# mantasu/face-crop-plus

Hardware: AMD Instinct MI355X
Metric: faces/sec end-to-end (detect+align+crop) (higher is better)
Workload: dtype f16x3; 1 GPU; RetinaFace detect + 5-pt align/crop, batch=32/GPU synthetic 1024x1024 RGB, strategy=largest, det_threshold=0.6, output 256x256, detector on 2 HIP streams x 16 images; global_batch=32, image_size=1024, parallelism=dp1

## Files before the change

### face-crop-plus_amd/csrc/fcp_conv_common.h

```cpp
#pragma once
#include <type_traits>
#include "fcp_common.h"
#include "fcp_hip.h"

typedef float f32x16 __attribute__((ext_vector_type(16)));
typedef float f32x4 __attribute__((ext_vector_type(4)));


constexpr int FCP_AUX_A = 0;
constexpr int FCP_AUX_B = 0;

namespace fcp_conv {

constexpr int BM = 128;
constexpr int BK = 32;

struct ConvK {
  const float* in;
  const float* w;
  const float* bias;
  float* out;
  const float* res1;
  const float* res2;
  int n, in_h, in_w, ph, pw, cin, in_ld, in_up2;
  int cout, kh, kw, stride, pad, out_h, out_w, out_ld;
  int pad_h;
  int M, ktiles, ctiles, wrow;
  float act_slope, alpha, alpha2;
  int res1_pre, res1_ld, res1_h, res1_w, res1_resize, res2_ld;
  float res1_sh, res1_sw;
  int grid_m, grid_n, vec_ok;
  unsigned in_bytes, w_bytes;
  const float* wscale;
  int in_fmt, out_fmt, res1_fmt, res2_fmt;
  const float* in2;
  unsigned in2_bytes;
  int csplit, in2_ld, ph2, pw2, stride2;
  int nt_store;
  int balance, cu_budget;
  int mfull, tail_rows, round_size;
  int big_tiles;
  int big_persist;
};


struct TapPiece {
  unsigned base, mask;
};

template <bool CIN4>
__device__ __forceinline__ TapPiece make_tap_piece(const ConvK& p, unsigned pbase, int hi0, int wi0, unsigned chan_off) {
  TapPiece t;
  t.base = ((pbase + (unsigned)(hi0 * p.pw + wi0)) * (unsigned)p.in_ld + chan_off) * 4u;
  t.mask = 0u;
  const int taps = CIN4 ? p.kh : p.kh * p.kw;
  for (int q = 0; q < taps; ++q) {
    const int kh_i = CIN4 ? q : q / p.kw;
    const int kw_i = CIN4 ? 0 : q - kh_i * p.kw;
    const bool ok = (unsigned)(hi0 + kh_i) < (unsigned)p.in_h && (unsigned)(wi0 + kw_i) < (unsigned)p.in_w;
    t.mask |= ok ? (1u << q) : 0u;
  }
  return t;
}

typedef unsigned int u32x4_t __attribute__((ext_vector_type(4)));
typedef _Float16 f16x2_t __attribute__((ext_vector_type(2)));
typedef _Float16 f16x8 __attribute__((ext_vector_type(8)));


__device__ __forceinline__ int xcd_tile_order(int nb, int bid) {
  const int q8 = nb >> 3, r8 = nb & 7, xcd = bid & 7;
  return (xcd < r8 ? xcd * (q8 + 1) : r8 * (q8 + 1) + (xcd - r8) * q8) + (bid >> 3);
}

template <typename M>
__device__ __forceinline__ void conv_out_pixel(const ConvK& p, M m, int hw, int& ni, int& ho, int& wo) {
  ni = (int)(m / hw);
  const int rem = (int)(m - (M)ni * hw);
  ho = rem / p.out_w;
  wo = rem - ho * p.out_w;
}

struct ConvRow {
  int ni;
  unsigned pbase;
  int hi0, wi0;
  unsigned base2;
};
__device__ __forceinline__ ConvRow conv_row(const ConvK& p, int m, int m_end, int hw, unsigned chan_off2) {
  ConvRow r = {0, 0u, -(1 << 28), 0, 0xFFFFFFFFu};
  if (m < m_end) {
    int ho, wo;
    conv_out_pixel(p, m, hw, r.ni, ho, wo);
    r.pbase = (unsigned)(r.ni * p.ph * p.pw);
    r.hi0 = ho * p.stride - p.pad_h;
    r.wi0 = wo * p.stride - p.pad;
    if (p.in2 != nullptr)
      r.base2 = (((unsigned)(r.ni * p.ph2 + ho * p.stride2) * (unsigned)p.pw2 + (unsigned)(wo * p.stride2)) * (unsigned)p.in2_ld + chan_off2) * 4u;
  }
  return r;
}

struct RowPiece {
  unsigned pbase;
  int hi0, wi0;
  int col;
  unsigned chan_off;
  TapPiece tp;
};
template <bool CIN4>
__device__ __forceinline__ RowPiece make_row_piece(const ConvK& p, const ConvRow& r, int col, unsigned chan_off) {
  RowPiece c = {r.pbase, r.hi0, r.wi0, CIN4 ? col : 0, CIN4 ? 0u : chan_off, {0u, 0u}};
  c.tp = make_tap_piece<CIN4>(p, c.pbase, c.hi0, c.wi0 + c.col, c.chan_off);
  return c;
}

struct TapWalk {
  int tap = 0, kh_i = 0, kw_i = 0, c0 = 0;
  template <bool CIN4>
  __device__ __forceinline__ void advance(const ConvK& p) {
    ++tap;
    if (CIN4) {
      ++kh_i;
    } else if (++kw_i >= p.kw) {
      kw_i = 0;
      if (++kh_i >= p.kh) { kh_i = 0; tap = 0; c0 += BK; }
    }
  }
};

template <bool CIN4, bool UP2, int NP>
__device__ __forceinline__ void set_tap(const ConvK& p, const TapWalk& t, const RowPiece (&pc)[NP], unsigned (&rowoff)[NP]) {
  if (UP2 && p.in_up2) {
#pragma unroll
    for (int i = 0; i < NP; ++i) {
      int hi = pc[i].hi0 + t.kh_i;
      int wi = pc[i].wi0 + (CIN4 ? pc[i].col : t.kw_i);
      const bool ok = (unsigned)hi < (unsigned)p.in_h && (unsigned)wi < (unsigned)p.in_w;
      hi >>= 1; wi >>= 1;
      const unsigned pix = pc[i].pbase + (unsigned)(hi * p.pw + wi);
      rowoff[i] = ok ? (pix * (unsigned)p.in_ld + pc[i].chan_off) * 4u : 0xFFFFFFFFu;
    }
  } else {
    const unsigned tapoff = (unsigned)((t.kh_i * p.pw + t.kw_i) * p.in_ld) * 4u;
#pragma unroll
    for (int i = 0; i < NP; ++i) rowoff[i] = ((pc[i].tp.mask >> t.tap) & 1u) ? pc[i].tp.base + tapoff : 0xFFFFFFFFu;
  }
}
template <bool CIN4, bool UP2, int NP>
__device__ __forceinline__ void next_tap(const ConvK& p, TapWalk& t, const RowPiece (&pc)[NP], unsigned (&rowoff)[NP]) {
  t.advance<CIN4>(p);
  set_tap<CIN4, UP2>(p, t, pc, rowoff);
}

__device__ __forceinline__ f32x4 buf_load16(__amdgpu_buffer_rsrc_t rsrc, unsigned voff) {
  return __builtin_bit_cast(f32x4, __builtin_amdgcn_raw_buffer_load_b128(rsrc, (int)voff, 0, 0));
}
__device__ __forceinline__ u32x4_t buf_load16u(__amdgpu_buffer_rsrc_t rsrc, unsigned voff) {
  return __builtin_bit_cast(u32x4_t, __builtin_amdgcn_raw_buffer_load_b128(rsrc, (int)voff, 0, 0));
}

template <int STEP, int A_LD, int B_LD>
__device__ __forceinline__ void dma_slice(const ConvK& p, __amdgpu_buffer_rsrc_t rs_in, __amdgpu_buffer_rsrc_t rs_in2, __amdgpu_buffer_rsrc_t rs_w,
                                          char* a, char* b, const unsigned (&rowoff)[A_LD], const unsigned (&base2)[A_LD],
                                          const unsigned (&woff)[B_LD], int c0, int kt) {
  constexpr int ROWB = 128;
  if (c0 >= p.csplit) {
#pragma unroll
    for (int i = 0; i < A_LD; ++i) {
      const unsigned ro = base2[i];
      __builtin_amdgcn_raw_ptr_buffer_load_lds(rs_in2, (__attribute__((address_space(3))) void*)(a + STEP * i * ROWB), 16,
                                               (int)(ro == 0xFFFFFFFFu ? 0xFFFFFFFFu : ro + (unsigned)((c0 - p.csplit) * 4)), 0, 0, FCP_AUX_A);
    }
  } else {
#pragma unroll
    for (int i = 0; i < A_LD; ++i) {
      const unsigned ro = rowoff[i];
      __builtin_amdgcn_raw_ptr_buffer_load_lds(rs_in, (__attribute__((address_space(3))) void*)(a + STEP * i * ROWB), 16,
                                               (int)(ro == 0xFFFFFFFFu ? 0xFFFFFFFFu : ro + (unsigned)(c0 * 4)), 0, 0, FCP_AUX_A);
    }
  }
#pragma unroll
  for (int i = 0; i < B_LD; ++i)
    __builtin_amdgcn_raw_ptr_buffer_load_lds(rs_w, (__attribute__((address_space(3))) void*)(b + STEP * i * ROWB), 16,
                                             (int)(woff[i] + (unsigned)(kt * BK * 4)), 0, 0, FCP_AUX_B);
}

__device__ __forceinline__ int swz(int row) { return ((row >> 1) & 7) ^ ((row & 1) << 2); }

__device__ __forceinline__ void frag_offsets(int lane, int (&offH)[2], int (&offL)[2]) {
  const int rsw = (((lane & 31) >> 1) & 7) ^ ((lane & 1) << 2);
  const int half = lane >> 5;
#pragma unroll
  for (int s = 0; s < 2; ++s) {
    offH[s] = ((2 * s + half) ^ rsw) << 4;
    offL[s] = ((4 + 2 * s + half) ^ rsw) << 4;
  }
}

template <int IMM>
__device__ __forceinline__ f16x8 lds_read128i(unsigned addr) {
  f16x8 v;
  asm volatile("ds_read_b128 %0, %1 offset:%2" : "=v"(v) : "v"(addr), "n"(IMM));
  return v;
}

template <int TM, int TN>
__device__ __forceinline__ void clear_acc(f32x16 (&acc)[TM][TN]) {
#pragma unroll
  for (int i = 0; i < TM; ++i)
#pragma unroll
    for (int j = 0; j < TN; ++j)
#pragma unroll
      for (int e = 0; e < 16; ++e) acc[i][j][e] = 0.f;
}

template <int HI>
__device__ __forceinline__ float fcp_mix_sum(unsigned h, unsigned l) {
  float r;
  const float one = 1.0f;
  if constexpr (HI) asm("v_fma_mix_f32 %0, %1, %2, %3 op_sel:[1,0,1] op_sel_hi:[1,0,1]" : "=v"(r) : "v"(h), "s"(one), "v"(l));
  else asm("v_fma_mix_f32 %0, %1, %2, %3 op_sel:[0,0,0] op_sel_hi:[1,0,1]" : "=v"(r) : "v"(h), "s"(one), "v"(l));
  return r;
}
template <int HI>
__device__ __forceinline__ float fcp_mix_diff(float x, unsigned h) {
  float r;
  const float minus_one = -1.0f;
  if constexpr (HI) asm("v_fma_mix_f32 %0, %1, %2, %3 op_sel:[1,0,0] op_sel_hi:[1,0,0]" : "=v"(r) : "v"(h), "s"(minus_one), "v"(x));
  else asm("v_fma_mix_f32 %0, %1, %2, %3 op_sel:[0,0,0] op_sel_hi:[1,0,0]" : "=v"(r) : "v"(h), "s"(minus_one), "v"(x));
  return r;
}

__device__ __forceinline__ void split8(const f32x4& x0, const f32x4& x1, u32x4_t& hi, u32x4_t& lo) {
  const float x[8] = {x0[0], x0[1], x0[2], x0[3], x1[0], x1[1], x1[2], x1[3]};
#pragma unroll
  for (int q = 0; q < 4; ++q) {
    const unsigned hu = __builtin_bit_cast(unsigned, __builtin_amdgcn_cvt_pkrtz(x[2 * q], x[2 * q + 1]));
    const float r0 = fcp_mix_diff<0>(x[2 * q], hu);
    const float r1 = fcp_mix_diff<1>(x[2 * q + 1], hu);
    hi[q] = hu;
    lo[q] = __builtin_bit_cast(unsigned, __builtin_amdgcn_cvt_pkrtz(r0, r1));
  }
}
__device__ __forceinline__ void split2(float x0, float x1, unsigned& hu, unsigned& lu) {
  hu = __builtin_bit_cast(unsigned, __builtin_amdgcn_cvt_pkrtz(x0, x1));
  lu = __builtin_bit_cast(unsigned, __builtin_amdgcn_cvt_pkrtz(fcp_mix_diff<0>(x0, hu), fcp_mix_diff<1>(x1, hu)));
}
__device__ __forceinline__ void join8(const u32x4_t& hi, const u32x4_t& lo, float (&x)[8]) {
#pragma unroll
  for (int q = 0; q < 4; ++q) {
    const unsigned hu = hi[q], lu = lo[q];
    x[2 * q] = fcp_mix_sum<0>(hu, lu);
    x[2 * q + 1] = fcp_mix_sum<1>(hu, lu);
  }
}
__device__ __forceinline__ long split_chan_off(int c) { return (long)(c >> 5) * 128 + (c & 31) * 2; }

__device__ __forceinline__ void load8(const float* base, long pix, int ld, int c, int fmt, float (&x)[8]) {
  if (fmt == 1) {
    const char* pb = reinterpret_cast<const char*>(base) + pix * ld * 4 + split_chan_off(c);
    join8(*reinterpret_cast<const u32x4_t*>(pb), *reinterpret_cast<const u32x4_t*>(pb + 64), x);
  } else {
    const f32x4 a = *reinterpret_cast<const f32x4*>(base + pix * ld + c);
    const f32x4 b = *reinterpret_cast<const f32x4*>(base + pix * ld + c + 4);
    x[0] = a[0]; x[1] = a[1]; x[2] = a[2]; x[3] = a[3]; x[4] = b[0]; x[5] = b[1]; x[6] = b[2]; x[7] = b[3];
  }
}

__device__ __forceinline__ void pack8(const float (&v)[8], int fmt, u32x4_t& a, u32x4_t& b) {
  if (fmt == 1) {
    split8(f32x4{v[0], v[1], v[2], v[3]}, f32x4{v[4], v[5], v[6], v[7]}, a, b);
  } else {
    a = __builtin_bit_cast(u32x4_t, f32x4{v[0], v[1], v[2], v[3]});
    b = __builtin_bit_cast(u32x4_t, f32x4{v[4], v[5], v[6], v[7]});
  }
}
__device__ __forceinline__ void store8(float* base, long pix, int ld, int c, int fmt, int nt, const u32x4_t& a, const u32x4_t& b) {
  if (fmt == 1) {
    char* ob = reinterpret_cast<char*>(base) + pix * ld * 4 + split_chan_off(c);
    if (nt) {
      __builtin_nontemporal_store(a, reinterpret_cast<u32x4_t*>(ob));
      __builtin_nontemporal_store(b, reinterpret_cast<u32x4_t*>(ob + 64));
    } else {
      *reinterpret_cast<u32x4_t*>(ob) = a;
      *reinterpret_cast<u32x4_t*>(ob + 64) = b;
    }
  } else {
    float* dst = base + pix * ld + c;
    *reinterpret_cast<u32x4_t*>(dst) = a;
    *reinterpret_cast<u32x4_t*>(dst + 4) = b;
  }
}
__device__ __forceinline__ void pack_store8(float* base, long pix, int ld, int c, int fmt, int nt, const float (&v)[8]) {
  u32x4_t a, b;
  if (fmt == 1) {
    pack8(v, 1, a, b);
    store8(base, pix, ld, c, 1, nt, a, b);
  } else {
    pack8(v, 0, a, b);
    store8(base, pix, ld, c, 0, 0, a, b);
  }
}

__device__ __forceinline__ float conv_scale_bias(float acc, float ws, float b) { return acc * ws + b; }

struct ConvEpi {
  bool res1, res1_pre, res2;
  float act_slope, alpha, alpha2;
};
template <typename E>
__device__ __forceinline__ float conv_finish(const E e, float x, float r1, float r2) {
  if (e.res1 && e.res1_pre) x += r1;
  x = x >= 0.f ? x : x * e.act_slope;
  x = x * e.alpha;
  if (e.res1 && !e.res1_pre) x += r1;
  if (e.res2) x = x * e.alpha2 + r2;
  return x;
}
template <typename E>
__device__ __forceinline__ float conv_value(const E& e, float acc, float ws, float b, float r1, float r2) {
  return conv_finish(e, conv_scale_bias(acc, ws, b), r1, r2);
}
__device__ __forceinline__ float conv_finish_relu(float x) { return conv_finish(ConvEpi{false, false, false, 0.f, 1.f, 1.f}, x, 0.f, 0.f); }
__device__ __forceinline__ float conv_finish_relu(float x, float r1) { return conv_finish(ConvEpi{true, true, false, 0.f, 1.f, 1.f}, x, r1, 0.f); }
__device__ __forceinline__ float conv_value_relu(float acc, float ws, float b) { return conv_finish_relu(conv_scale_bias(acc, ws, b)); }

__device__ __forceinline__ long res1_pixel(const ConvK& p, long m, int hw) {
  int ni, ho, wo;
  conv_out_pixel(p, m, hw, ni, ho, wo);
  int sh = (int)floorf(ho * p.res1_sh);
  int sw = (int)floorf(wo * p.res1_sw);
  sh = sh < p.res1_h - 1 ? sh : p.res1_h - 1;
  sw = sw < p.res1_w - 1 ? sw : p.res1_w - 1;
  return ((long)ni * p.res1_h + sh) * p.res1_w + sw;
}

__device__ __forceinline__ constexpr int mfma_c_row(int rr, int half) { return (rr & 3) + 8 * (rr >> 2) + 4 * half; }

template <int BN, int TM, int TN, int WTM, int WTN>
__device__ __forceinline__ void stage_acc_tile(const f32x16 (&acc)[TM][TN], float* Cs, int lane, int wm, int wn) {
  const int half = lane >> 5;
#pragma unroll
  for (int i = 0; i < TM; ++i)
#pragma unroll
    for (int j = 0; j < TN; ++j)
#pragma unroll
      for (int rr = 0; rr < 16; ++rr) {
        const int row = wm * WTM + i * 32 + mfma_c_row(rr, half);
        Cs[row * BN + wn * WTN + j * 32 + (lane & 31)] = acc[i][j][rr];
      }
  __syncthreads();
}

template <int BN, int TM, int TN, int WTM, int WTN>
__device__ __forceinline__ void conv_epilogue(const ConvK& p, f32x16 (&acc)[TM][TN], float* smem, int tile_m,
                                              int tile_n, int tid, int lane, int wm, int wn, int hw) {
  constexpr int CPR = BN / 4;
  constexpr int RPP = 256 / CPR;
  constexpr int PASSES = BM / RPP;
  float* Cs = smem;
  const int ccol = (tid % CPR) * 4;
  const int crow = tid / CPR;
  const int co = tile_n * BN + ccol;
  const bool vec = p.vec_ok && (co + 3 < p.cout);
  const long m0 = (long)tile_m * BM + crow;

  const bool pre1 = p.res1 != nullptr && !p.res1_resize && vec;
  const bool pre2 = p.res2 != nullptr && vec;
  stage_acc_tile<BN, TM, TN, WTM, WTN>(acc, Cs, lane, wm, wn);

  f32x4 bias4 = {0.f, 0.f, 0.f, 0.f}, ws4 = {1.f, 1.f, 1.f, 1.f};
  if (p.bias != nullptr) {
#pragma unroll
    for (int e = 0; e < 4; ++e)
      if (co + e < p.cout) bias4[e] = p.bias[co + e];
  }
  if (p.wscale != nullptr) {
#pragma unroll
    for (int e = 0; e < 4; ++e)
      if (co + e < p.cout) ws4[e] = p.wscale[co + e];
  }
  constexpr int EPC = PASSES < 4 ? PASSES : 4;
#pragma unroll 1
  for (int g = 0; g < PASSES; g += EPC) {
    f32x4 r1v[EPC], r2v[EPC];
    if (pre1) {
#pragma unroll
      for (int i = 0; i < EPC; ++i) {
        const long m = m0 + (long)(g + i) * RPP;
        r1v[i] = m < p.M ? *reinterpret_cast<const f32x4*>(p.res1 + m * p.res1_ld + co) : f32x4{0.f, 0.f, 0.f, 0.f};
      }
    }
    if (pre2) {
#pragma unroll
      for (int i = 0; i < EPC; ++i) {
        const long m = m0 + (long)(g + i) * RPP;
        r2v[i] = m < p.M ? *reinterpret_cast<const f32x4*>(p.res2 + m * p.res2_ld + co) : f32x4{0.f, 0.f, 0.f, 0.f};
      }
    }
#pragma unroll
    for (int i = 0; i < EPC; ++i) {
      const int row = crow + (g + i) * RPP;
      const long m = m0 + (long)(g + i) * RPP;
      if (m >= p.M || co >= p.cout) continue;
      f32x4 v = *reinterpret_cast<const f32x4*>(Cs + row * BN + ccol);
      f32x4 r1 = {0.f, 0.f, 0.f, 0.f}, r2 = {0.f, 0.f, 0.f, 0.f};
      if (pre1) {
        r1 = r1v[i];
      } else if (p.res1 != nullptr) {
        const long roff = (p.res1_resize ? res1_pixel(p, m, hw) : m) * p.res1_ld + co;
        if (vec) {
          r1 = *reinterpret_cast<const f32x4*>(p.res1 + roff);
        } else {
#pragma unroll
          for (int e = 0; e < 4; ++e)
            if (co + e < p.cout) r1[e] = p.res1[roff + e];
        }
      }
      if (pre2) {
        r2 = r2v[i];
      } else if (p.res2 != nullptr) {
#pragma unroll
        for (int e = 0; e < 4; ++e)
          if (co + e < p.cout) r2[e] = p.res2[m * p.res2_ld + co + e];
      }
#pragma unroll
      for (int e = 0; e < 4; ++e) v[e] = conv_value(p, v[e], ws4[e], bias4[e], r1[e], r2[e]);
      float* dst = p.out + m * p.out_ld + co;
      if (vec) {
        *reinterpret_cast<f32x4*>(dst) = v;
      } else {
#pragma unroll
        for (int e = 0; e < 4; ++e)
          if (co + e < p.cout) dst[e] = v[e];
      }
    }
  }
}


template <int I, int N, typename F>
__device__ __forceinline__ void fcp_static_for(F&& f) {
  if constexpr (I < N) {
    f(std::integral_constant<int, I>{});
    fcp_static_for<I + 1, N>(f);
  }
}

template <int TM, int TN, int WTM, int WTN>
__device__ __forceinline__ void conv_epilogue_regs(const ConvK& p, f32x16 (&acc)[TM][TN], int m_start, int m_end, int tm_act, int co_tile,
                                                   int co_end, int wm, int wn, int lane, int hw) {
    const int lp = lane & 15, lg = lane >> 4;
  auto swap32 = [](float& x, float& y) {
    const auto r = __builtin_amdgcn_permlane32_swap(__float_as_uint(x), __float_as_uint(y), false, false);
    const unsigned r0 = r[0], r1 = r[1];
    x = __uint_as_float(r0); y = __uint_as_float(r1);
  };
  auto swap16 = [](float& x, float& y) {
    const auto r = __builtin_amdgcn_permlane16_swap(__float_as_uint(x), __float_as_uint(y), false, false);
    const unsigned r0 = r[0], r1 = r[1];
    x = __uint_as_float(r0); y = __uint_as_float(r1);
  };
  constexpr int GI = TM < 2 ? TM : 2;
  constexpr int NGI = (TM + GI - 1) / GI;
  constexpr int NG = TN * NGI;
  u32x4_t pend_a[GI][2], pend_b[GI][2];
  auto row_of = [&](int i, int set) { return m_start + wm * WTM + i * 32 + 16 * set + lp; };
  auto chan_of = [&](int jj) { return co_tile + wn * WTN + jj * 32 + 8 * lg; };
  auto flush = [&](auto gc) {
    constexpr int g = decltype(gc)::value, jj = g / NGI, i0 = (g % NGI) * GI;
    const int co = chan_of(jj);
    fcp_static_for<0, GI>([&](auto ic) {
      constexpr int i = i0 + decltype(ic)::value;
      if constexpr (i < TM) {
        fcp_static_for<0, 2>([&](auto sc) {
          constexpr int set = decltype(sc)::value;
          const int mi = row_of(i, set);
          if (i < tm_act && mi < m_end && co < co_end) store8(p.out, mi, p.out_ld, co, p.out_fmt, 0, pend_a[i - i0][set], pend_b[i - i0][set]);
        });
      }
    });
  };
  fcp_static_for<0, NG>([&](auto gc) {
    constexpr int g = decltype(gc)::value, j = g / NGI, i0 = (g % NGI) * GI;
    const int co = chan_of(j);
    const bool cok = co < co_end;
    const int cc = cok ? co : co_tile;
    u32x4_t r1a[GI][2], r1b[GI][2];
    if (p.res1 != nullptr) {
      fcp_static_for<0, GI>([&](auto ic) {
        constexpr int i = i0 + decltype(ic)::value;
        if constexpr (i < TM) {
          fcp_static_for<0, 2>([&](auto sc) {
            constexpr int set = decltype(sc)::value;
            const int mi = row_of(i, set);
            const long m = (i < tm_act && mi < m_end && cok) ? (long)mi : (long)m_start;
            const long rpix = p.res1_resize ? res1_pixel(p, m, hw) : m;
            if (p.res1_fmt == 1) {
              const char* pb = reinterpret_cast<const char*>(p.res1) + rpix * p.res1_ld * 4 + split_chan_off(cc);
              r1a[i - i0][set] = *reinterpret_cast<const u32x4_t*>(pb);
              r1b[i - i0][set] = *reinterpret_cast<const u32x4_t*>(pb + 64);
            } else {
              r1a[i - i0][set] = *reinterpret_cast<const u32x4_t*>(p.res1 + rpix * p.res1_ld + cc);
              r1b[i - i0][set] = *reinterpret_cast<const u32x4_t*>(p.res1 + rpix * p.res1_ld + cc + 4);
            }
          });
        }
      });
    }
    __builtin_amdgcn_sched_barrier(0);
    if constexpr (g > 0) flush(std::integral_constant<int, g - 1>{});
    __builtin_amdgcn_sched_barrier(0);
    float bias8[8], ws8[8];
    {
      const f32x4 w0 = *reinterpret_cast<const f32x4*>(p.wscale + cc), w1 = *reinterpret_cast<const f32x4*>(p.wscale + cc + 4);
      f32x4 b0 = {0.f, 0.f, 0.f, 0.f}, b1 = b0;
      if (p.bias != nullptr) { b0 = *reinterpret_cast<const f32x4*>(p.bias + cc); b1 = *reinterpret_cast<const f32x4*>(p.bias + cc + 4); }
#pragma unroll
      for (int e = 0; e < 4; ++e) { ws8[e] = w0[e]; ws8[4 + e] = w1[e]; bias8[e] = b0[e]; bias8[4 + e] = b1[e]; }
    }
    fcp_static_for<0, GI>([&](auto ic) {
      constexpr int i = i0 + decltype(ic)::value;
      if constexpr (i < TM) {
        float va[8], vb[8];
        fcp_static_for<0, 4>([&](auto ec) {
          constexpr int e = decltype(ec)::value;
          float q0 = acc[i][j][e], q1 = acc[i][j][4 + e], q2 = acc[i][j][8 + e], q3 = acc[i][j][12 + e];
          swap32(q0, q1);
          swap32(q2, q3);
          swap32(q0, q2); swap16(q0, q2);
          swap32(q1, q3); swap16(q1, q3);
          va[e] = q0; va[4 + e] = q1; vb[e] = q2; vb[4 + e] = q3;
        });
        fcp_static_for<0, 2>([&](auto sc) {
          constexpr int set = decltype(sc)::value;
          float (&v)[8] = set == 0 ? va : vb;
          float r1[8], r2[8];
          if (p.res1 != nullptr) {
            if (p.res1_fmt == 1) {
              join8(r1a[i - i0][set], r1b[i - i0][set], r1);
            } else {
              const f32x4 fa = __builtin_bit_cast(f32x4, r1a[i - i0][set]), fb = __builtin_bit_cast(f32x4, r1b[i - i0][set]);
              r1[0] = fa[0]; r1[1] = fa[1]; r1[2] = fa[2]; r1[3] = fa[3]; r1[4] = fb[0]; r1[5] = fb[1]; r1[6] = fb[2]; r1[7] = fb[3];
            }
          }
          if (p.res2 != nullptr) {
            const int mi = row_of(i, set);
            load8(p.res2, (i < tm_act && mi < m_end && cok) ? (long)mi : (long)m_start, p.res2_ld, cc, p.res2_fmt, r2);
          }
#pragma unroll
          for (int e = 0; e < 8; ++e) v[e] = conv_value(p, v[e], ws8[e], bias8[e], r1[e], r2[e]);
          pack8(v, p.out_fmt, pend_a[i - i0][set], pend_b[i - i0][set]);
        });
      }
    });
  });
  flush(std::integral_constant<int, NG - 1>{});
}

template <int BN, int TM, int TN, int WTM, int WTN>
__device__ __forceinline__ void conv_epilogue8(const ConvK& p, f32x16 (&acc)[TM][TN], float* smem, int tile_m,
                                               int tile_n, int tid, int lane, int wm, int wn, int hw) {
  constexpr int CPR = BN / 8;
  constexpr int RPP = 256 / CPR;
  constexpr int PASSES = BM / RPP;
  float* Cs = smem;
  const int ccol = (tid % CPR) * 8;
  const int crow = tid / CPR;
  const int co = tile_n * BN + ccol;
  const long m0 = (long)tile_m * BM + crow;
  stage_acc_tile<BN, TM, TN, WTM, WTN>(acc, Cs, lane, wm, wn);
  if (co >= p.cout) return;
  float bias8[8], ws8[8];
#pragma unroll
  for (int e = 0; e < 8; ++e) {
    bias8[e] = p.bias != nullptr ? p.bias[co + e] : 0.f;
    ws8[e] = p.wscale != nullptr ? p.wscale[co + e] : 1.f;
  }
#pragma unroll
  for (int g = 0; g < PASSES; ++g) {
    const int row = crow + g * RPP;
    const long m = m0 + (long)g * RPP;
    if (m >= p.M) continue;
    float v[8], r1[8], r2[8];
    {
      const f32x4 a = *reinterpret_cast<const f32x4*>(Cs + row * BN + ccol);
      const f32x4 b = *reinterpret_cast<const f32x4*>(Cs + row * BN + ccol + 4);
      v[0] = a[0]; v[1] = a[1]; v[2] = a[2]; v[3] = a[3]; v[4] = b[0]; v[5] = b[1]; v[6] = b[2]; v[7] = b[3];
    }
    if (p.res1 != nullptr) load8(p.res1, p.res1_resize ? res1_pixel(p, m, hw) : m, p.res1_ld, co, p.res1_fmt, r1);
    if (p.res2 != nullptr) load8(p.res2, m, p.res2_ld, co, p.res2_fmt, r2);
#pragma unroll
    for (int e = 0; e < 8; ++e) v[e] = conv_value(p, v[e], ws8[e], bias8[e], r1[e], r2[e]);
    pack_store8(p.out, m, p.out_ld, co, p.out_fmt, p.nt_store, v);
  }
}

int launch_f16x3(const ConvK& k, int tile_n, bool cin4, hipStream_t s);
int launch_f16x3_dma(const ConvK& k, int tile_n, hipStream_t s);
int launch_f16x3_halo(const ConvK& k, hipStream_t s);
int launch_f16x3_halo_wide(const ConvK& k, hipStream_t s);
int launch_f16x3_big(const ConvK& k, int tile_n, hipStream_t s);

}
```

### face-crop-plus_amd/csrc/fcp_conv_f16x3_big.hip

```cpp
#include "fcp_conv_common.h"

#include <type_traits>

using namespace fcp_conv;

namespace {

constexpr int BMB = 256;
constexpr int NT = 512;
constexpr int ROWB = 128;
constexpr int STAGE = 1 << 16;

template <int BN>
__global__ void __launch_bounds__(NT, 1) conv_igemm_f16x3_big(const ConvK p) {
  constexpr int WAVES_N = BN == 256 ? 4 : 2;
  constexpr int WAVES_M = 8 / WAVES_N;
  constexpr int WTM = BMB / WAVES_M, WTN = BN / WAVES_N;
  constexpr int TM = WTM / 32, TN = WTN / 32;
  constexpr int A_LD = BMB / 64, B_LD = BN / 64;

  extern __shared__ __attribute__((aligned(16))) float smem[];
  char* lds = reinterpret_cast<char*>(smem);

  const int nb = p.big_tiles;
  int vb = blockIdx.x;
  int tile_n = 0, m_start = 0, m_end = 0;
  auto decode = [&](int bid) {
    const int rbase = (bid / p.round_size) * p.round_size;
    const int nr = nb - rbase < p.round_size ? nb - rbase : p.round_size;
    const int bi = bid - rbase;
    const int logical = rbase + xcd_tile_order(nr, bi);
    tile_n = logical % p.grid_n;
    const int tile_m = logical / p.grid_n;
    m_start = tile_m < p.mfull ? tile_m * BMB : p.mfull * BMB + (tile_m - p.mfull) * p.tail_rows;
    const int m_rows = tile_m < p.mfull ? BMB : p.tail_rows;
    m_end = m_start + m_rows < p.M ? m_start + m_rows : p.M;
  };
  decode(vb);

  const int tid = threadIdx.x;
  const int lane = tid & 63;
  const int wave_u = __builtin_amdgcn_readfirstlane(tid >> 6);
  const int wm = wave_u / WAVES_N, wn = wave_u % WAVES_N;
  const int lrow = tid >> 3;
  const int csrc = (tid & 7) ^ (((lrow >> 1) & 7) ^ ((lrow & 1) << 2));

  const int hw = p.out_h * p.out_w;
  RowPiece pc[A_LD];
  unsigned base2[A_LD];
  unsigned rowoff[A_LD], woff[B_LD];
  auto setup_tile = [&]() {
#pragma unroll
    for (int i = 0; i < A_LD; ++i) {
      const int m = m_start + lrow + 64 * i;
      unsigned pbase = 0;
      int hi0 = -(1 << 28), wi0 = 0;
      base2[i] = 0xFFFFFFFFu;
      if (m < m_end) {
        int ni, ho, wo;
        conv_out_pixel(p, m, hw, ni, ho, wo);
        pbase = (unsigned)(ni * p.ph * p.pw);
        hi0 = ho * p.stride - p.pad_h;
        wi0 = wo * p.stride - p.pad;
        if (p.in2 != nullptr)
          base2[i] = (((unsigned)(ni * p.ph2 + ho * p.stride2) * (unsigned)p.pw2 + (unsigned)(wo * p.stride2)) * (unsigned)p.in2_ld +
                      (unsigned)(csrc * 4)) * 4u;
      }
      pc[i].tp = make_tap_piece<false>(p, pbase, hi0, wi0, (unsigned)(csrc * 4));
    }
#pragma unroll
    for (int i = 0; i < B_LD; ++i) woff[i] = (unsigned)(((tile_n * BN + lrow + 64 * i) * p.wrow + csrc * 4) * 4);
  };
  setup_tile();
  __amdgpu_buffer_rsrc_t rs_in2 = __builtin_amdgcn_make_buffer_rsrc(const_cast<float*>(p.in2 ? p.in2 : p.in), 0, p.in2_bytes, 0x00020000);
  __amdgpu_buffer_rsrc_t rs_in = __builtin_amdgcn_make_buffer_rsrc(const_cast<float*>(p.in), 0, p.in_bytes, 0x00020000);
  __amdgpu_buffer_rsrc_t rs_w = __builtin_amdgcn_make_buffer_rsrc(const_cast<float*>(p.w), 0, p.w_bytes, 0x00020000);
  TapWalk tw;
  auto advance = [&]() { next_tap<false, false>(p, tw, pc, rowoff); };
  auto dma = [&](int kt, int stage) {
    char* a = lds + stage * STAGE + wave_u * 8 * ROWB;
    dma_slice<64>(p, rs_in, rs_in2, rs_w, a, a + BMB * ROWB, rowoff, base2, woff, tw.c0, kt);
  };

  f32x16 acc[TM][TN];

  const unsigned lds0 = (unsigned)(size_t)(__attribute__((address_space(3))) char*)lds;
  int offH[2], offL[2];
  frag_offsets(lane, offH, offL);
  const unsigned arow = lds0 + (unsigned)((wm * WTM + (lane & 31)) * ROWB);
  const unsigned brow = lds0 + (unsigned)((BMB + wn * WTN + (lane & 31)) * ROWB);
  unsigned aH[2], aL[2], bH[2], bL[2];
#pragma unroll
  for (int s = 0; s < 2; ++s) {
    aH[s] = arow + (unsigned)offH[s]; aL[s] = arow + (unsigned)offL[s];
    bH[s] = brow + (unsigned)offH[s]; bL[s] = brow + (unsigned)offL[s];
  }

  auto prefetch_tile = [&]() {
    tw = TapWalk();
    set_tap<false, false>(p, tw, pc, rowoff);
    dma(0, 0);
    if (p.ktiles > 1) {
      advance();
      dma(1, 1);
    }
  };
  prefetch_tile();
  int tm_act = 0;
  auto main_loop = [&](auto tma_c) {
    constexpr int TMA = decltype(tma_c)::value;
    f16x8 fah[2][TMA > 0 ? TMA : 1], fal[2][TMA > 0 ? TMA : 1], fbh[2][TN], fbl[2][TN];
  auto read_frags = [&](auto set_c, unsigned stage_xor) {
    constexpr int set = decltype(set_c)::value;
    fcp_static_for<0, TMA>([&](auto ic) {
      constexpr int i = decltype(ic)::value;
      fah[set][i] = lds_read128i<i * 32 * ROWB>(aH[set] ^ stage_xor);
      fal[set][i] = lds_read128i<i * 32 * ROWB>(aL[set] ^ stage_xor);
    });
    fcp_static_for<0, TN>([&](auto jc) {
      constexpr int j = decltype(jc)::value;
      fbh[set][j] = lds_read128i<j * 32 * ROWB>(bH[set] ^ stage_xor);
      fbl[set][j] = lds_read128i<j * 32 * ROWB>(bL[set] ^ stage_xor);
    });
  };
  constexpr std::integral_constant<int, 0> SET0{};
  constexpr std::integral_constant<int, 1> SET1{};
  auto mfmas_reads = [&](auto cs_c, auto ls_c, unsigned stage_xor) {
    constexpr int cs = decltype(cs_c)::value, ls = decltype(ls_c)::value;
    constexpr int NM = 3 * TMA * TN, NR = 2 * TMA + 2 * TN;
    fcp_static_for<0, NM>([&](auto mc) {
      constexpr int m = decltype(mc)::value;
      constexpr int g = m / (TMA * TN), i = (m % (TMA * TN)) / TN, j = m % TN;
      if constexpr (g == 0) acc[i][j] = __builtin_amdgcn_mfma_f32_32x32x16_f16(fbh[cs][j], fal[cs][i], acc[i][j], 0, 0, 0);
      else if constexpr (g == 1) acc[i][j] = __builtin_amdgcn_mfma_f32_32x32x16_f16(fbl[cs][j], fah[cs][i], acc[i][j], 0, 0, 0);
      else acc[i][j] = __builtin_amdgcn_mfma_f32_32x32x16_f16(fbh[cs][j], fah[cs][i], acc[i][j], 0, 0, 0);
      __builtin_amdgcn_sched_barrier(0);
      fcp_static_for<0, NR>([&](auto rc) {
        constexpr int r = decltype(rc)::value;
        if constexpr (((r + 1) * NM) / NR - 1 == m
        ) {
          if constexpr (r < 2 * TMA) {
            constexpr int ii = r / 2;
            if constexpr (r % 2 == 0) fah[ls][ii] = lds_read128i<ii * 32 * ROWB>(aH[ls] ^ stage_xor);
            else fal[ls][ii] = lds_read128i<ii * 32 * ROWB>(aL[ls] ^ stage_xor);
          } else {
            constexpr int jj = (r - 2 * TMA) / 2;
            if constexpr (r % 2 == 0) fbh[ls][jj] = lds_read128i<jj * 32 * ROWB>(bH[ls] ^ stage_xor);
            else fbl[ls][jj] = lds_read128i<jj * 32 * ROWB>(bL[ls] ^ stage_xor);
          }
          __builtin_amdgcn_sched_barrier(0);
        }
      });
    });
  };

  read_frags(SET0, 0u);
  asm volatile("s_waitcnt lgkmcnt(0)" ::: "memory");
  __builtin_amdgcn_sched_barrier(0);

  unsigned sx = 0u;
  for (int kt = 0; kt < p.ktiles; ++kt) {
    mfmas_reads(SET0, SET1, sx);
    __builtin_amdgcn_sched_barrier(0);
    asm volatile("s_waitcnt lgkmcnt(0)" ::: "memory");
    asm volatile("s_waitcnt vmcnt(0)" ::: "memory");
    __builtin_amdgcn_s_barrier();
    __builtin_amdgcn_sched_barrier(0);
    const bool dma_first = wave_u >= 4;
    if (dma_first && kt + 2 < p.ktiles) {
      advance();
      dma(kt + 2, kt & 1);
    }
    __builtin_amdgcn_sched_barrier(0);
    mfmas_reads(SET1, SET0, sx ^ (unsigned)STAGE);
    __builtin_amdgcn_sched_barrier(0);
    if (!dma_first && kt + 2 < p.ktiles) {
      advance();
      dma(kt + 2, kt & 1);
    }
    __builtin_amdgcn_sched_barrier(0);
    asm volatile("s_waitcnt lgkmcnt(0)" ::: "memory");
    __builtin_amdgcn_sched_barrier(0);
    sx ^= (unsigned)STAGE;
  }
  };
  for (;;) {
  asm volatile("s_waitcnt vmcnt(0)" ::: "memory");
  __builtin_amdgcn_s_barrier();
  __builtin_amdgcn_sched_barrier(0);
  tm_act = (m_end - m_start - wm * WTM + 31) >> 5;
  tm_act = __builtin_amdgcn_readfirstlane(tm_act < 0 ? 0 : (tm_act > TM ? TM : tm_act));
  clear_acc(acc);
  fcp_static_for<0, TM + 1>([&](auto tc) {
    if (tm_act == decltype(tc)::value) main_loop(tc);
  });
  asm volatile("s_waitcnt vmcnt(0)" ::: "memory");
  __builtin_amdgcn_s_barrier();

  const int e_tile_n = tile_n, e_m_start = m_start, e_m_end = m_end, e_tm_act = tm_act;
  const bool more = p.big_persist && vb + p.round_size < nb;
  if (more) {
    vb += p.round_size;
    decode(vb);
    setup_tile();
    prefetch_tile();
  }
  conv_epilogue_regs<TM, TN, WTM, WTN>(p, acc, e_m_start, e_m_end, e_tm_act, e_tile_n * BN,
                                       (e_tile_n + 1) * BN < p.cout ? (e_tile_n + 1) * BN : p.cout, wm, wn, lane, hw);
  if (!more) break;
  }
}

template <int BN>
int launch(ConvK k, hipStream_t s) {
  const size_t lds = 2 * (size_t)STAGE;
  FCP_LDS_OPT_IN((&conv_igemm_f16x3_big<BN>), lds);
  k.grid_n = fcp_cdiv(k.cout, BN);
  int cus = k.cu_budget > 0 ? k.cu_budget : fcp_cu_count();
  cus = cus < 8 ? 8 : (cus & ~7);
  k.round_size = cus;
  const int mt = fcp_cdiv(k.M, BMB);
  k.mfull = mt;
  k.tail_rows = BMB;
  k.grid_m = mt;
  if (k.balance) {
    const long tiles = (long)mt * k.grid_n;
    const long full_rounds = tiles / cus;
    const int mfull = (int)((full_rounds * cus) / k.grid_n);
    const long rem = (long)k.M - (long)mfull * BMB;
    if (rem > 0) {
      const long slots = cus / k.grid_n > 0 ? cus / k.grid_n : 1;
      long r = ((rem + slots - 1) / slots + 31) / 32 * 32;
      r = r < 32 ? 32 : r;
      if (r < BMB) {
        k.mfull = mfull;
        k.tail_rows = (int)r;
        k.grid_m = mfull + (int)((rem + r - 1) / r);
      }
    }
  }
  k.big_tiles = k.grid_m * k.grid_n;
  static const int persist_env = getenv("FCP_BIG_PERSIST") ? atoi(getenv("FCP_BIG_PERSIST")) : -1;
  k.big_persist = persist_env < 0 ? (k.cu_budget == 0) : (persist_env != 0);
  hipLaunchKernelGGL((conv_igemm_f16x3_big<BN>), dim3(k.big_persist && k.big_tiles > k.round_size ? k.round_size : k.big_tiles), dim3(NT), lds, s, k);
  FCP_LAUNCH_OK();
  return 0;
}

}

namespace fcp_conv {

int launch_f16x3_big(const ConvK& k, int tile_n, hipStream_t s) {
  return tile_n == 256 ? launch<256>(k, s) : tile_n == 192 ? launch<192>(k, s) : launch<128>(k, s);
}

}
```

Before: 1482 faces/s.

## Add strip-based input reuse path for 3x3 stride-1 convs in big igemm kernel

Adds a STRIP variant of the big implicit-GEMM conv kernel for 3x3/stride1/pad1 convolutions with widths 64 or 128. It loads a padded row strip of input into LDS once per (kh, channel chunk) and reuses it across the three kw taps by shifting LDS read addresses, instead of re-DMAing the A tile for every tap. Filter slices get their own smaller double-buffered stages. This cuts global-to-LDS traffic for A, at the cost of more complex addressing, larger LDS use and stricter shape conditions.

```diff
diff --git a/face-crop-plus_amd/csrc/fcp_conv_common.h b/face-crop-plus_amd/csrc/fcp_conv_common.h
--- a/face-crop-plus_amd/csrc/fcp_conv_common.h
+++ b/face-crop-plus_amd/csrc/fcp_conv_common.h
@@ -187,6 +187,63 @@
 }
 
 __device__ __forceinline__ int swz(int row) { return ((row >> 1) & 7) ^ ((row & 1) << 2); }
+
+constexpr int STRIP_PAD = 16;
+constexpr int STRIP_LD = 6;
+constexpr int STRIP_BYTES = 384 * 128;
+
+__device__ __forceinline__ TapPiece make_strip_piece(const ConvK& p, int q, int ni0, int rem0, int rows, int hw, int wsh, unsigned chan_off) {
+  TapPiece t = {0u, 0u};
+  const int pitch = p.out_w + STRIP_PAD;
+  const int rr = (int)(((float)q + 0.5f) * (1.0f / (float)pitch));
+  const int cc = q - rr * pitch - 1;
+  const int dm = rr << wsh;
+  if (dm < rows && (unsigned)cc < (unsigned)p.in_w) {
+    const bool next = rem0 + dm >= hw;
+    const int ni = next ? ni0 + 1 : ni0;
+    const int hi0 = ((next ? rem0 + dm - hw : rem0 + dm) >> wsh) - p.pad_h;
+    t.base = (((unsigned)(ni * p.ph * p.pw) + (unsigned)(hi0 * p.pw + cc)) * (unsigned)p.in_ld + chan_off) * 4u;
+#pragma unroll
+    for (int k = 0; k < 3; ++k) t.mask |= (unsigned)(hi0 + k) < (unsigned)p.in_h ? (1u << k) : 0u;
+  }
+  return t;
+}
+
+__device__ __forceinline__ unsigned strip_run_mask(const ConvK& p, int wave_u, int rows) {
+  const int pitch = p.out_w + STRIP_PAD;
+  unsigned m = 0u;
+#pragma unroll
+  for (int i = 0; i < STRIP_LD; ++i) {
+    const int q0 = 64 * i + 8 * wave_u;
+    m |= (q0 < rows && q0 % pitch < p.out_w + 2) ? (1u << i) : 0u;
+  }
+  return m;
+}
+
+__device__ __forceinline__ void dma_strip(const ConvK& p, __amdgpu_buffer_rsrc_t rs_in, char* a, const unsigned (&base)[STRIP_LD], unsigned mask,
+                                          unsigned runs, int kh_i, int c0) {
+  const unsigned khoff = (unsigned)(kh_i * p.pw * p.in_ld + c0) * 4u;
+  const unsigned mk = mask >> kh_i;
+#pragma unroll
+  for (int i = 0; i < STRIP_LD; ++i) {
+    if ((runs >> i) & 1u)
+      __builtin_amdgcn_raw_ptr_buffer_load_lds(rs_in, (__attribute__((address_space(3))) void*)(a + 64 * i * 128), 16,
+                                               (int)((mk & (1u << (3 * i))) ? base[i] + khoff : 0xFFFFFFFFu), 0, 0, FCP_AUX_A);
+  }
+}
+
+template <int STEP, int B_LD>
+__device__ __forceinline__ void dma_filter_slice(__amdgpu_buffer_rsrc_t rs_w, char* b, const unsigned (&woff)[B_LD], int kt) {
+#pragma unroll
+  for (int i = 0; i < B_LD; ++i)
+    __builtin_amdgcn_raw_ptr_buffer_load_lds(rs_w, (__attribute__((address_space(3))) void*)(b + STEP * i * 128), 16,
+                                             (int)(woff[i] + (unsigned)(kt * BK * 4)), 0, 0, FCP_AUX_B);
+}
+
+__device__ __forceinline__ unsigned strip_tap_term(int l31, int kw, unsigned hb) {
+  const unsigned t = (unsigned)(l31 + kw);
+  return ((t << 7) | (((t << 3) & 0x70u) ^ ((t & 1u) << 6))) ^ hb;
+}
 
 __device__ __forceinline__ void frag_offsets(int lane, int (&offH)[2], int (&offL)[2]) {
   const int rsw = (((lane & 31) >> 1) & 7) ^ ((lane & 1) << 2);
diff --git a/face-crop-plus_amd/csrc/fcp_conv_f16x3_big.hip b/face-crop-plus_amd/csrc/fcp_conv_f16x3_big.hip
--- a/face-crop-plus_amd/csrc/fcp_conv_f16x3_big.hip
+++ b/face-crop-plus_amd/csrc/fcp_conv_f16x3_big.hip
@@ -10,8 +10,12 @@
 constexpr int NT = 512;
 constexpr int ROWB = 128;
 constexpr int STAGE = 1 << 16;
-
-template <int BN>
+constexpr int FSTAGE = 1 << 15;
+constexpr int STRIP0 = 2 * FSTAGE;
+constexpr int STRIP_LDS = STRIP0 + 2 * STRIP_BYTES;
+static_assert(STRIP_LDS <= 160 * 1024, "LDS budget");
+
+template <int BN, bool STRIP>
 __global__ void __launch_bounds__(NT, 1) conv_igemm_f16x3_big(const ConvK p) {
   constexpr int WAVES_N = BN == 256 ? 4 : 2;
   constexpr int WAVES_M = 8 / WAVES_N;
@@ -46,10 +50,25 @@
   const int csrc = (tid & 7) ^ (((lrow >> 1) & 7) ^ ((lrow & 1) << 2));
 
   const int hw = p.out_h * p.out_w;
-  RowPiece pc[A_LD];
-  unsigned base2[A_LD];
-  unsigned rowoff[A_LD], woff[B_LD];
+  RowPiece pc[STRIP ? 1 : A_LD];
+  unsigned base2[STRIP ? 1 : A_LD];
+  unsigned rowoff[STRIP ? 1 : A_LD], woff[B_LD];
+  unsigned sbase[STRIP_LD], smask = 0u;
+  const int wsh = STRIP ? __builtin_ctz((unsigned)p.out_w) : 0;
+  const unsigned sruns = STRIP ? __builtin_amdgcn_readfirstlane(strip_run_mask(p, wave_u, BMB + STRIP_PAD * (BMB >> wsh))) : 0u;
   auto setup_tile = [&]() {
+    if constexpr (STRIP) {
+      const int ni0 = m_start / hw;
+      int lr = lrow;
+      asm volatile("" : "+v"(lr));
+      smask = 0u;
+#pragma unroll
+      for (int i = 0; i < STRIP_LD; ++i) {
+        const TapPiece t = make_strip_piece(p, lr + 64 * i, ni0, m_start - ni0 * hw, m_end - m_start, hw, wsh, (unsigned)(csrc * 4));
+        sbase[i] = t.base;
+        smask |= t.mask << (3 * i);
+      }
+    } else {
 #pragma unroll
     for (int i = 0; i < A_LD; ++i) {
       const int m = m_start + lrow + 64 * i;
@@ -68,6 +87,7 @@
       }
       pc[i].tp = make_tap_piece<false>(p, pbase, hi0, wi0, (unsigned)(csrc * 4));
     }
+    }
 #pragma unroll
     for (int i = 0; i < B_LD; ++i) woff[i] = (unsigned)(((tile_n * BN + lrow + 64 * i) * p.wrow + csrc * 4) * 4);
   };
@@ -76,10 +96,19 @@
   __amdgpu_buffer_rsrc_t rs_in = __builtin_amdgcn_make_buffer_rsrc(const_cast<float*>(p.in), 0, p.in_bytes, 0x00020000);
   __amdgpu_buffer_rsrc_t rs_w = __builtin_amdgcn_make_buffer_rsrc(const_cast<float*>(p.w), 0, p.w_bytes, 0x00020000);
   TapWalk tw;
-  auto advance = [&]() { next_tap<false, false>(p, tw, pc, rowoff); };
+  auto advance = [&]() {
+    if constexpr (STRIP) tw.advance<false>(p);
+    else next_tap<false, false>(p, tw, pc, rowoff);
+  };
   auto dma = [&](int kt, int stage) {
-    char* a = lds + stage * STAGE + wave_u * 8 * ROWB;
-    dma_slice<64>(p, rs_in, rs_in2, rs_w, a, a + BMB * ROWB, rowoff, base2, woff, tw.c0, kt);
+    if constexpr (STRIP) {
+      if (tw.kw_i == 0)
+        dma_strip(p, rs_in, lds + STRIP0 + (((tw.c0 >> 5) + tw.kh_i) & 1) * STRIP_BYTES + wave_u * 8 * ROWB, sbase, smask, sruns, tw.kh_i, tw.c0);
+      dma_filter_slice<64>(rs_w, lds + stage * FSTAGE + wave_u * 8 * ROWB, woff, kt);
+    } else {
+      char* a = lds + stage * STAGE + wave_u * 8 * ROWB;
+      dma_slice<64>(p, rs_in, rs_in2, rs_w, a, a + BMB * ROWB, rowoff, base2, woff, tw.c0, kt);
+    }
   };
 
   f32x16 acc[TM][TN];
@@ -88,7 +117,13 @@
   int offH[2], offL[2];
   frag_offsets(lane, offH, offL);
   const unsigned arow = lds0 + (unsigned)((wm * WTM + (lane & 31)) * ROWB);
-  const unsigned brow = lds0 + (unsigned)((BMB + wn * WTN + (lane & 31)) * ROWB);
+  const unsigned brow = lds0 + (unsigned)(((STRIP ? 0 : BMB) + wn * WTN + (lane & 31)) * ROWB);
+  constexpr unsigned BSTAGE = STRIP ? FSTAGE : STAGE;
+  const unsigned hb = (unsigned)(lane >> 5) << 4;
+  auto strip_sub = [&](int i) {
+    const int r0 = wm * WTM + 32 * i;
+    return (unsigned)((r0 + STRIP_PAD * (r0 >> wsh)) * ROWB);
+  };
   unsigned aH[2], aL[2], bH[2], bL[2];
 #pragma unroll
   for (int s = 0; s < 2; ++s) {
@@ -98,7 +133,7 @@
 
   auto prefetch_tile = [&]() {
     tw = TapWalk();
-    set_tap<false, false>(p, tw, pc, rowoff);
+    if constexpr (!STRIP) set_tap<false, false>(p, tw, pc, rowoff);
     dma(0, 0);
     if (p.ktiles > 1) {
       advance();
@@ -110,12 +145,24 @@
   auto main_loop = [&](auto tma_c) {
     constexpr int TMA = decltype(tma_c)::value;
     f16x8 fah[2][TMA > 0 ? TMA : 1], fal[2][TMA > 0 ? TMA : 1], fbh[2][TN], fbl[2][TN];
-  auto read_frags = [&](auto set_c, unsigned stage_xor) {
+  auto read_a = [&](auto set_c, auto ic, auto lo_c, unsigned stage_xor, unsigned sb, unsigned th, unsigned tl) {
+    constexpr int set = decltype(set_c)::value, i = decltype(ic)::value, lo = decltype(lo_c)::value;
+    if constexpr (STRIP) {
+      const unsigned a = ((lo ? tl : th) ^ (unsigned)(32 * set)) + (sb + strip_sub(i));
+      if constexpr (lo) fal[set][i] = lds_read128i<0>(a);
+      else fah[set][i] = lds_read128i<0>(a);
+    } else {
+      if constexpr (lo) fal[set][i] = lds_read128i<i * 32 * ROWB>(aL[set] ^ stage_xor);
+      else fah[set][i] = lds_read128i<i * 32 * ROWB>(aH[set] ^ stage_xor);
+    }
+  };
+  constexpr std::integral_constant<int, 0> HI{};
+  constexpr std::integral_constant<int, 1> LO{};
+  auto read_frags = [&](auto set_c, unsigned stage_xor, unsigned sb, unsigned th, unsigned tl) {
     constexpr int set = decltype(set_c)::value;
     fcp_static_for<0, TMA>([&](auto ic) {
-      constexpr int i = decltype(ic)::value;
-      fah[set][i] = lds_read128i<i * 32 * ROWB>(aH[set] ^ stage_xor);
-      fal[set][i] = lds_read128i<i * 32 * ROWB>(aL[set] ^ stage_xor);
+      read_a(set_c, ic, HI, stage_xor, sb, th, tl);
+      read_a(set_c, ic, LO, stage_xor, sb, th, tl);
     });
     fcp_static_for<0, TN>([&](auto jc) {
       constexpr int j = decltype(jc)::value;
@@ -125,7 +172,7 @@
   };
   constexpr std::integral_constant<int, 0> SET0{};
   constexpr std::integral_constant<int, 1> SET1{};
-  auto mfmas_reads = [&](auto cs_c, auto ls_c, unsigned stage_xor) {
+  auto mfmas_reads = [&](auto cs_c, auto ls_c, unsigned stage_xor, unsigned sb, unsigned th, unsigned tl) {
     constexpr int cs = decltype(cs_c)::value, ls = decltype(ls_c)::value;
     constexpr int NM = 3 * TMA * TN, NR = 2 * TMA + 2 * TN;
     fcp_static_for<0, NM>([&](auto mc) {
@@ -140,9 +187,7 @@
         if constexpr (((r + 1) * NM) / NR - 1 == m
         ) {
           if constexpr (r < 2 * TMA) {
-            constexpr int ii = r / 2;
-            if constexpr (r % 2 == 0) fah[ls][ii] = lds_read128i<ii * 32 * ROWB>(aH[ls] ^ stage_xor);
-            else fal[ls][ii] = lds_read128i<ii * 32 * ROWB>(aL[ls] ^ stage_xor);
+            read_a(ls_c, std::integral_constant<int, r / 2>{}, std::integral_constant<int, r % 2>{}, stage_xor, sb, th, tl);
           } else {
             constexpr int jj = (r - 2 * TMA) / 2;
             if constexpr (r % 2 == 0) fbh[ls][jj] = lds_read128i<jj * 32 * ROWB>(bH[ls] ^ stage_xor);
@@ -154,13 +199,18 @@
     });
   };
 
-  read_frags(SET0, 0u);
+  const unsigned strip0 = lds0 + (unsigned)STRIP0;
+  unsigned sb_cur = strip0, sb_nxt = strip0;
+  int kw_nxt = 1;
+  unsigned th_cur = STRIP ? strip_tap_term(lane & 31, 0, hb) : 0u, th_nxt = STRIP ? strip_tap_term(lane & 31, 1, hb) : 0u;
+  unsigned tl_cur = th_cur ^ 64u, tl_nxt = th_nxt ^ 64u;
+  read_frags(SET0, 0u, sb_cur, th_cur, tl_cur);
   asm volatile("s_waitcnt lgkmcnt(0)" ::: "memory");
   __builtin_amdgcn_sched_barrier(0);
 
   unsigned sx = 0u;
   for (int kt = 0; kt < p.ktiles; ++kt) {
-    mfmas_reads(SET0, SET1, sx);
+    mfmas_reads(SET0, SET1, sx, sb_cur, th_cur, tl_cur);
     __builtin_amdgcn_sched_barrier(0);
     asm volatile("s_waitcnt lgkmcnt(0)" ::: "memory");
     asm volatile("s_waitcnt vmcnt(0)" ::: "memory");
@@ -172,7 +222,7 @@
       dma(kt + 2, kt & 1);
     }
     __builtin_amdgcn_sched_barrier(0);
-    mfmas_reads(SET1, SET0, sx ^ (unsigned)STAGE);
+    mfmas_reads(SET1, SET0, sx ^ BSTAGE, sb_nxt, th_nxt, tl_nxt);
     __builtin_amdgcn_sched_barrier(0);
     if (!dma_first && kt + 2 < p.ktiles) {
       advance();
@@ -181,7 +231,13 @@
     __builtin_amdgcn_sched_barrier(0);
     asm volatile("s_waitcnt lgkmcnt(0)" ::: "memory");
     __builtin_amdgcn_sched_barrier(0);
-    sx ^= (unsigned)STAGE;
+    sx ^= BSTAGE;
+    if constexpr (STRIP) {
+      sb_cur = sb_nxt; th_cur = th_nxt; tl_cur = tl_nxt;
+      if (++kw_nxt == 3) { kw_nxt = 0; sb_nxt = sb_nxt == strip0 ? strip0 + (unsigned)STRIP_BYTES : strip0; }
+      th_nxt = strip_tap_term(lane & 31, kw_nxt, hb);
+      tl_nxt = th_nxt ^ 64u;
+    }
   }
   };
   for (;;) {
@@ -213,8 +269,8 @@
 
 template <int BN>
 int launch(ConvK k, hipStream_t s) {
-  const size_t lds = 2 * (size_t)STAGE;
-  FCP_LDS_OPT_IN((&conv_igemm_f16x3_big<BN>), lds);
+  FCP_LDS_OPT_IN((&conv_igemm_f16x3_big<BN, false>), 2 * (size_t)STAGE);
+  FCP_LDS_OPT_IN((&conv_igemm_f16x3_big<BN, true>), (size_t)STRIP_LDS);
   k.grid_n = fcp_cdiv(k.cout, BN);
   int cus = k.cu_budget > 0 ? k.cu_budget : fcp_cu_count();
   cus = cus < 8 ? 8 : (cus & ~7);
@@ -242,7 +298,13 @@
   k.big_tiles = k.grid_m * k.grid_n;
   static const int persist_env = getenv("FCP_BIG_PERSIST") ? atoi(getenv("FCP_BIG_PERSIST")) : -1;
   k.big_persist = persist_env < 0 ? (k.cu_budget == 0) : (persist_env != 0);
-  hipLaunchKernelGGL((conv_igemm_f16x3_big<BN>), dim3(k.big_persist && k.big_tiles > k.round_size ? k.round_size : k.big_tiles), dim3(NT), lds, s, k);
+  const char* strip_env = getenv("FCP_BIG_STRIP");
+  const bool strip_ok = k.kh == 3 && k.kw == 3 && k.stride == 1 && k.pad == 1 && k.in2 == nullptr && !k.in_up2 && k.in_w == k.out_w &&
+                        (k.out_w == 32 || k.out_w == 64 || k.out_w == 128) && (k.out_h * k.out_w) % BMB == 0 && k.tail_rows % k.out_w == 0;
+  const bool strip = strip_ok && (strip_env != nullptr ? atoi(strip_env) != 0 : k.out_w >= 64);
+  const dim3 grid(k.big_persist && k.big_tiles > k.round_size ? k.round_size : k.big_tiles);
+  if (strip) hipLaunchKernelGGL((conv_igemm_f16x3_big<BN, true>), grid, dim3(NT), (size_t)STRIP_LDS, s, k);
+  else hipLaunchKernelGGL((conv_igemm_f16x3_big<BN, false>), grid, dim3(NT), 2 * (size_t)STAGE, s, k);
   FCP_LAUNCH_OK();
   return 0;
 }
```

Result: no change. 1487 faces/s, median of 6 (+0.3%).
